# Traneptora/jxlatte

Hardware: AMD Instinct MI355X
Metric: Mpixels/s decoded (VarDCT 4K frame) at 1/2/4/8 MI355X vs host-CPU jxlatte (higher is better)
Workload: dtype f32; 1 GPU; vardct4k: 8 independent 3840x2160 VarDCT frames per GPU (mix=default, Gab + EPF x2 + XYB, f32 out), inputs resident in HBM; frames_per_gpu=8, frames_total=8, frame_seeds=1000 + i, frame i on rank i mod 1, distinct_frames=8, streams=2, kernel_launches_per_frame=2

## Files before the change

jxlatte_amd/csrc/restore_fused_body.h:

```cpp
#pragma once
#include <hip/hip_ext.h>
#include "jxl_internal.h"
#include <algorithm>
#include "restore_sink.h"
#include "epf_quot3.h"
#include <cstdlib>
#include <type_traits>

namespace jxl {

#ifndef JXL_EPF3_PH2_WAVES
#define JXL_EPF3_PH2_WAVES 2
#endif

namespace {

__device__ __forceinline__ int mirror_c(int c, int size) {
    while (c < 0 || c >= size) {
        const int tc = ~c;
        c = tc >= 0 ? tc : (size << 1) + tc;
    }
    return c;
}

template <bool GAB, int ITERS>
struct Geo {
    static constexpr int RG = GAB ? 1 : 0;
    static constexpr int R0 = (ITERS == 3 || ITERS == 4) ? 3 : 0;
    static constexpr int R1 = (ITERS >= 1 && ITERS <= 3) ? 2 : 0;
    static constexpr int R2 = (ITERS == 2 || ITERS == 3) ? 1 : 0;
    static constexpr int SHR = ITERS == 3 ? (R1 + R2) : ITERS == 2 ? R2 : 0;
#ifndef JXL_EPF0_WH
#define JXL_EPF0_WH 64
#endif
    static constexpr int WH = ITERS == 4 ? JXL_EPF0_WH : 32;
    static constexpr int OW = 64 - 2 * SHR, OH = WH - 2 * SHR;
    static constexpr int RE = R0 + R1 + R2;
    static constexpr int RT = RE + RG;
    static constexpr int IW = OW + 2 * RT, IH = OH + 2 * RT;
    static constexpr int SW = IW + 3;
    static constexpr int SH = IH + 1;
    static constexpr int PLANE = SW * SH;
    static constexpr size_t LDS_BYTES = sizeof(float) * (3 * PLANE + 16 * 16);
};

template <int PS>
__device__ __forceinline__ float adiff(const float* p, int u, int v, float s) {
    return u < v ? fabsf(p[u] - p[v]) * s : fabsf(p[v] - p[u]) * s;
}

template <int ITER, int SW, int PLANE, int PH, bool PLAINDIV = false, bool CHAINS = true>
__device__ __forceinline__ void epf_patch(const float* __restrict__ src, int ry, int rx, const float* s_inv ,
                                          const float* bmul , const EpfParams& ep, float res[3][4 * PH]) {
    constexpr int NP = 4 * PH;
    constexpr int R = ITER == 0 ? 3 : ITER == 1 ? 2 : 1;
    constexpr int NW = 4 + 2 * R, NH = PH + 2 * R;
    constexpr int NT = ITER == 0 ? 12 : 4;
    constexpr int TY[12] = {0, 0, -1, 1, -1, 1, 1, -1, 0, 0, 2, -2};
    constexpr int TX[12] = {-1, 1, 0, 0, 1, 1, -1, -1, -2, 2, 0, 0};
    constexpr int QY[5] = {0, 0, 0, -1, 1};
    constexpr int QX[5] = {0, -1, 1, 0, 0};

    float dist[NP][NT];
#pragma unroll
    for (int i = 0; i < NP; i++)
#pragma unroll
        for (int t = 0; t < NT; t++) dist[i][t] = 0.0f;

    if (ITER != 0 && CHAINS) {
        float hc[PH][5], vc[PH + 1][4];
        auto chain_channel = [&](int c, auto first_channel) {
            constexpr bool FIRST = decltype(first_channel)::value;
            float nb[NH * NW];
            const float* pc = src + c * PLANE + (ry - R) * SW + (rx - R);
#pragma unroll
            for (int y = 0; y < NH; y++)
#pragma unroll
                for (int x = 0; x < NW; x++) nb[y * NW + x] = pc[y * SW + x];
            const float sc = ep.channel_scale[c];
#pragma unroll
            for (int py = 0; py < PH; py++)
#pragma unroll
                for (int j = 0; j < 5; j++) {
                    const int cy = py + R, cx = j - 1 + R;
                    if (ITER == 2) {
                        const float t = adiff<NW>(nb, cy * NW + cx, cy * NW + cx + 1, sc);
                        hc[py][j] = FIRST ? t : hc[py][j] + t;
                    } else
#pragma unroll
                        for (int q = 0; q < 5; q++) {
                            const int u = (cy + QY[q]) * NW + cx + QX[q];
                            const float t = adiff<NW>(nb, u, u + 1, sc);
                            hc[py][j] = (FIRST && q == 0) ? t : hc[py][j] + t;
                        }
                }
            constexpr int I0 = 0;
#pragma unroll
            for (int i = I0; i <= PH; i++)
#pragma unroll
                for (int px = 0; px < 4; px++) {
                    const int cy = i - 1 + R, cx = px + R;
                    if (ITER == 2) {
                        const float t = adiff<NW>(nb, cy * NW + cx, (cy + 1) * NW + cx, sc);
                        vc[i][px] = FIRST ? t : vc[i][px] + t;
                    } else
#pragma unroll
                        for (int q = 0; q < 5; q++) {
                            const int u = (cy + QY[q]) * NW + cx + QX[q];
                            const float t = adiff<NW>(nb, u, u + NW, sc);
                            vc[i][px] = (FIRST && q == 0) ? t : vc[i][px] + t;
                        }
                }
        };
        chain_channel(0, std::true_type{});
#pragma unroll 1
        for (int c = 1; c < 3; c++) chain_channel(c, std::false_type{});
#pragma unroll
        for (int py = 0; py < PH; py++)
#pragma unroll
            for (int px = 0; px < 4; px++) {
                dist[py * 4 + px][0] = hc[py][px];
                dist[py * 4 + px][1] = hc[py][px + 1];
                dist[py * 4 + px][2] = vc[py][px];
                dist[py * 4 + px][3] = vc[py + 1][px];
            }
    } else {
    constexpr bool HROW = ITER == 0 && CHAINS && PH == 1;
    float h1[5], h2[6];
#pragma unroll
    for (int j = 0; j < 5; j++) h1[j] = 0.0f;
#pragma unroll
    for (int j = 0; j < 6; j++) h2[j] = 0.0f;
#pragma unroll 1
    for (int c = 0; c < 3; c++) {
        float nb[NH * NW];
        const float* pc = src + c * PLANE + (ry - R) * SW + (rx - R);
#pragma unroll
        for (int y = 0; y < NH; y++)
#pragma unroll
            for (int x = 0; x < NW; x++) nb[y * NW + x] = pc[y * SW + x];
        const float sc = ep.channel_scale[c];
#pragma unroll
        for (int py = 0; py < PH; py++)
#pragma unroll
            for (int px = 0; px < 4; px++) {
                const int cy = py + R, cx = px + R;
#pragma unroll
                for (int t = 0; t < NT; t++) {
                    if (HROW && TY[t] == 0) continue;
                    if (ITER == 2) {
                        dist[py * 4 + px][t] =
                            dist[py * 4 + px][t] + adiff<NW>(nb, cy * NW + cx, (cy + TY[t]) * NW + cx + TX[t], sc);
                    } else {
#pragma unroll
                        for (int q = 0; q < 5; q++) {
                            const int u = (cy + QY[q]) * NW + cx + QX[q];
                            const int v = (cy + TY[t] + QY[q]) * NW + cx + TX[t] + QX[q];
                            dist[py * 4 + px][t] = dist[py * 4 + px][t] + adiff<NW>(nb, u, v, sc);
                        }
                    }
                }
            }
        if (HROW) {
            constexpr int cy = R;
#pragma unroll
            for (int j = 0; j < 5; j++)
#pragma unroll
                for (int q = 0; q < 5; q++) {
                    const int u = (cy + QY[q]) * NW + (j - 1 + R) + QX[q];
                    h1[j] = h1[j] + adiff<NW>(nb, u, u + 1, sc);
                }
#pragma unroll
            for (int j = 0; j < 6; j++)
#pragma unroll
                for (int q = 0; q < 5; q++) {
                    const int u = (cy + QY[q]) * NW + (j - 2 + R) + QX[q];
                    h2[j] = h2[j] + adiff<NW>(nb, u, u + 2, sc);
                }
        }
    }
    if (HROW) {
#pragma unroll
        for (int px = 0; px < 4; px++)
#pragma unroll
            for (int t = 0; t < NT; t++) {
                if (TY[t] != 0) continue;
                dist[px][t] = TX[t] == -1 ? h1[px] : TX[t] == 1 ? h1[px + 1] : TX[t] == -2 ? h2[px] : h2[px + 2];
            }
    }
    }
    float sumW[NP];
    bool skip[NP];
#pragma unroll
    for (int i = 0; i < NP; i++) {
        const float s = s_inv[i];
        skip[i] = (s != s) || (s > (1.0f / 0.3f));
        float sw = 0.0f + 1.0f;
#pragma unroll
        for (int t = 0; t < NT; t++) {
            const float d = dist[i][t] * bmul[i];
            const float v = 1.0f - d * ep.sigma_scale * s;
            const float w = !PLAINDIV ? __builtin_fminf(__builtin_fmaxf(v, 0.0f), 1.0f) : __builtin_fmaxf(v, 0.0f);
            dist[i][t] = w;
            sw = sw + w;
        }
        sumW[i] = sw;
    }
    constexpr int RT2 = ITER == 0 ? 2 : 1;
    constexpr int MW = 4 + 2 * RT2, MH = PH + 2 * RT2;
    if constexpr (!PLAINDIV) {
        float num[3][NP];
#pragma unroll
        for (int c = 0; c < 3; c++) {
            float nb[MH * MW];
            const float* pc = src + c * PLANE + (ry - RT2) * SW + (rx - RT2);
#pragma unroll
            for (int y = 0; y < MH; y++)
#pragma unroll
                for (int x = 0; x < MW; x++) nb[y * MW + x] = pc[y * SW + x];
#pragma unroll
            for (int py = 0; py < PH; py++)
#pragma unroll
                for (int px = 0; px < 4; px++) {
                    const int i = py * 4 + px;
                    const int cy = py + RT2, cx = px + RT2;
                    float sc = 0.0f + nb[cy * MW + cx] * 1.0f;
#pragma unroll
                    for (int t = 0; t < NT; t++) sc = sc + nb[(cy + TY[t]) * MW + cx + TX[t]] * dist[i][t];
                    num[c][i] = sc;
                }
        }
        epf_quot3_patch<NP>(num, sumW, res, [&](int c, int i, float q) {
            const float s = s_inv[i];
            return ((s != s) || (s > (1.0f / 0.3f))) ? src[c * PLANE + (ry + i / 4) * SW + rx + i % 4] : q;
        });
        return;
    }
#pragma unroll
    for (int c = 0; c < 3; c++) {
        float nb[MH * MW];
        const float* pc = src + c * PLANE + (ry - RT2) * SW + (rx - RT2);
#pragma unroll
        for (int y = 0; y < MH; y++)
#pragma unroll
            for (int x = 0; x < MW; x++) nb[y * MW + x] = pc[y * SW + x];
#pragma unroll
        for (int py = 0; py < PH; py++)
#pragma unroll
            for (int px = 0; px < 4; px++) {
                const int i = py * 4 + px;
                const int cy = py + RT2, cx = px + RT2;
                float sc = 0.0f + nb[cy * MW + cx] * 1.0f;
#pragma unroll
                for (int t = 0; t < NT; t++) sc = sc + nb[(cy + TY[t]) * MW + cx + TX[t]] * dist[i][t];
#ifdef JXL_EPF_DIV_BRANCH
                res[c][i] = skip[i] ? nb[cy * MW + cx] : sc / sumW[i];
#else
                float qv = sc / sumW[i];
                asm volatile("" : "+v"(qv));
                res[c][i] = skip[i] ? nb[cy * MW + cx] : qv;
#endif
            }
    }
}

struct TileCtx {
    int ix0, iy0;
    int W, H;
    bool edge;
};

template <int PH, bool EDGE>
__device__ __forceinline__ void patch_sigma(int ry, int rx, const TileCtx& tc, const float* __restrict__ sig, int scy0, int scx0,
                                            const EpfParams& ep, float s_inv[4 * PH], float bmul[4 * PH]) {
    const int gx0 = tc.ix0 + rx;
    int cxa = (gx0 >> 3) - scx0, cxb = ((gx0 + 3) >> 3) - scx0;
    if (EDGE) {
        cxa = (min(max(gx0, 0), tc.W - 1) >> 3) - scx0;
        cxb = (min(max(gx0 + 3, 0), tc.W - 1) >> 3) - scx0;
    }
    const int first_n = 8 - (gx0 & 7);
    const uint32_t colb = 0x8181u >> (gx0 & 7);
#pragma unroll
    for (int py = 0; py < PH; py++) {
        const int gy = tc.iy0 + ry + py;
        const bool rowb = ((gy + 1) & 7) < 2;
        int crow = ((gy >> 3) - scy0) * 16;
        if (EDGE) crow = ((min(max(gy, 0), tc.H - 1) >> 3) - scy0) * 16;
        const float sa = sig[crow + cxa], sb = sig[crow + cxb];
        const uint32_t bm = rowb ? 0xfu : colb;
#pragma unroll
        for (int px = 0; px < 4; px++) {
            bmul[py * 4 + px] = (bm & (1u << px)) ? ep.border_sad_mul : 1.0f;
            s_inv[py * 4 + px] = px < first_n ? sa : sb;
        }
    }
}

template <int ITER, typename G, bool LAST, int PH, bool EDGE, bool PLAINDIV, typename Sink>
__device__ __forceinline__ void epf_stage(float* buf, int m, const TileCtx& tc, const float* __restrict__ sig, int scy0, int scx0,
                                          const EpfParams& ep, Sink sink) {
    constexpr int SW = G::SW, PLANE = G::PLANE;
    const int rw = G::IW - 2 * m, rh = G::IH - 2 * m;
    constexpr int NTHR = 512 / PH;
    const int pcols = (rw + 3) >> 2, prows = (rh + PH - 1) / PH;
    const int cblocks = (pcols + 7) >> 3, n_groups = cblocks * ((prows + 3) >> 2);
    const int q = threadIdx.x & 31;
    auto patch_of = [&](int g, int& prow, int& pcol) {
        pcol = (g % cblocks) * 8 + (q & 7);
        prow = (g / cblocks) * 4 + (q >> 3);
        return prow < prows && pcol < pcols;
    };
    if (LAST) {
        for (int g = threadIdx.x >> 5; g < n_groups; g += NTHR / 32) {
            int prow, pcol;
            if (!patch_of(g, prow, pcol)) continue;
            const int ry = m + prow * PH, rx = m + pcol * 4;
            float s_inv[4 * PH], bmul[4 * PH];
            patch_sigma<PH, EDGE>(ry, rx, tc, sig, scy0, scx0, ep, s_inv, bmul);
            float res[3][4 * PH];
            epf_patch<ITER, SW, PLANE, PH, PLAINDIV>(buf, ry, rx, s_inv, bmul, ep, res);
#pragma unroll
            for (int py = 0; py < PH; py++) {
                const int y = ry + py;
                if (y < G::IH - m) sink.row4(y, rx, &res[0][py * 4], &res[1][py * 4], &res[2][py * 4], min(4, G::IW - m - rx));
            }
        }
    } else {
        static_assert((64 / 4) * ((32 + PH - 1) / PH) <= NTHR, "one patch per thread");
        int prow, pcol;
        const bool act = patch_of(threadIdx.x >> 5, prow, pcol);
        const int ry = m + prow * PH, rx = m + pcol * 4;
        float res[3][4 * PH];
        if (act) {
            float s_inv[4 * PH], bmul[4 * PH];
            patch_sigma<PH, EDGE>(ry, rx, tc, sig, scy0, scx0, ep, s_inv, bmul);
            epf_patch<ITER, SW, PLANE, PH, PLAINDIV>(buf, ry, rx, s_inv, bmul, ep, res);
        }
        __syncthreads();
        if (act) {
#pragma unroll
            for (int py = 0; py < PH; py++) {
                const int y = ry + py;
#pragma unroll
                for (int px = 0; px < 4; px++) {
                    const int x = rx + px;
                    if (y < G::IH - m && x < G::IW - m) {
#pragma unroll
                        for (int c = 0; c < 3; c++) buf[c * PLANE + y * SW + x] = res[c][py * 4 + px];
                    }
                }
            }
        }
    }
}

template <typename G, int NTHR>
__device__ __forceinline__ void mirror_fixup(float* __restrict__ buf, int m, int rem, const TileCtx& tc) {
    const int rw = G::IW - 2 * m, rh = G::IH - 2 * m;
    __syncthreads();
    for (int i = threadIdx.x; i < rw * rh; i += NTHR) {
        const int y = m + i / rw, x = m + i % rw;
        const int gy = tc.iy0 + y, gx = tc.ix0 + x;
        const bool outside = gy < 0 || gy >= tc.H || gx < 0 || gx >= tc.W;
        const bool near = gy >= -rem && gy < tc.H + rem && gx >= -rem && gx < tc.W + rem;
        if (outside && near) {
            const int my = mirror_c(gy, tc.H) - tc.iy0, mx = mirror_c(gx, tc.W) - tc.ix0;
#pragma unroll
            for (int c = 0; c < 3; c++) buf[c * G::PLANE + y * G::SW + x] = buf[c * G::PLANE + my * G::SW + mx];
        }
    }
}


typedef float v2f_t __attribute__((ext_vector_type(2)));
struct __attribute__((packed, aligned(4))) f2a4 {
    float x, y;
};

template <int SK, bool NT = false, bool EDGE = true>
struct OutSink {
    const FusedArgs& a;
    const TileCtx& tc;
    __device__ __forceinline__ void colour(float& v0, float& v1, float& v2) const {
        if (a.p.xyb) invert_xyb_px(a.p.xybp, v0, v1, v2);
    }
    __device__ __forceinline__ void operator()(int y, int x, float v0, float v1, float v2) const {
        const int gy = tc.iy0 + y, gx = tc.ix0 + x;
        if (EDGE && (gy >= tc.H || gx >= tc.W)) return;
        colour(v0, v1, v2);
        sink_store_k<SK>(a, (uint32_t)(gy * tc.W + gx), v0, v1, v2);
    }
    __device__ __forceinline__ void row4(int y, int x, const float* r0, const float* r1, const float* r2, int nvalid) const {
        const int gy = tc.iy0 + y, gx = tc.ix0 + x;
        if (EDGE && gy >= tc.H) return;
        const int n = EDGE ? min(nvalid, tc.W - gx) : nvalid;
        if (n <= 0) return;
        float o[3][4];
#pragma unroll
        for (int i = 0; i < 4; i++) {
            o[0][i] = r0[i];
            o[1][i] = r1[i];
            o[2][i] = r2[i];
            colour(o[0][i], o[1][i], o[2][i]);
        }
        const uint32_t g = (uint32_t)(gy * tc.W + gx);
        if (n == 4 && (g & 1u) == 0 && sink_store4_k<SK, NT>(a, g, o)) return;
#pragma unroll
        for (int i = 0; i < 4; i++)
            if (i < n) sink_store_k<SK>(a, g + i, o[0][i], o[1][i], o[2][i]);
    }
};

template <bool GAB, int ITERS, int SK, int PH, bool EDGE, bool PLAINDIV>
__device__ __forceinline__ void restore_epf_stages(const FusedArgs& a, float* cur, int m, const TileCtx& tc, const float* __restrict__ sig,
                                                   int scy0, int scx0);

template <bool GAB, int ITERS, int SK, int PH, int LAY = 0, bool PLAINDIV = false>
__device__ __forceinline__ void restore_fused_body(const FusedArgs& a) {
    using G = Geo<GAB, ITERS>;
    constexpr int NTHR = 512 / PH;
    extern __shared__ float lds[];
    constexpr int FRONT = LAY == 1 ? 3 : 0;
    float* A = lds + FRONT;
    float* sig = lds + 3 * G::PLANE;
    const int W = a.W, H = a.H;
    TileCtx tc;
    tc.W = W;
    tc.H = H;
    const int tiles_x = (W + G::OW - 1) / G::OW, tiles_y = (H + G::OH - 1) / G::OH;
    int ox, oy;
    {
        const int n_tiles = tiles_x * tiles_y;
        const int per_xcd = (n_tiles + 7) >> 3;
        const int tile = (int)(blockIdx.x & 7u) * per_xcd + (int)(blockIdx.x >> 3);
        if (tile >= n_tiles) return;
        ox = (tile % tiles_x) * G::OW;
        oy = (tile / tiles_x) * G::OH;
    }
    tc.ix0 = ox - G::RT;
    tc.iy0 = oy - G::RT;
    tc.edge = tc.ix0 < 0 || tc.iy0 < 0 || tc.ix0 + G::IW > W || tc.iy0 + G::IH > H;

    const int scy0 = max(tc.iy0, 0) >> 3, scx0 = max(tc.ix0, 0) >> 3;
    if (ITERS > 0 && threadIdx.x < 256) {
        const int cy = scy0 + (threadIdx.x >> 4), cx = scx0 + (threadIdx.x & 15);
        float v = 0.0f;
        if (cy < ((H + 7) >> 3) && cx < a.bw) v = a.inv_sigma[cy * a.bw + cx];
        if (v != v || v > (1.0f / 0.3f)) v = __builtin_inff();
        sig[threadIdx.x] = v;
    }
    if (LAY == 1 && !tc.edge) {
        constexpr int NCX = (G::IW + 6) / 8 + 1, NCY = (G::IH + 6) / 8 + 1, TOTAL = NCX * NCY * 16;
        const int cells_w = W >> 3;
        const int ccy0 = tc.iy0 >> 3, ccx0 = tc.ix0 >> 3;
        static_assert(NTHR % 16 == 0, "a lane keeps its piece index");
        constexpr int CSTEP = NTHR / 16, DY = CSTEP / NCX, DX = CSTEP % NCX;
        const int pc = threadIdx.x & 15;
        const int cyi0 = (int)(threadIdx.x >> 4) / NCX;
        int cxi = (int)(threadIdx.x >> 4) - cyi0 * NCX;
        int y = ((ccy0 + cyi0) << 3) + (pc >> 1) - tc.iy0, x = ((ccx0 + cxi) << 3) + ((pc & 1) << 2) - tc.ix0;
        const size_t tile0 = (size_t)(uint32_t)(ccy0 * cells_w + ccx0) << 6;
        const char* const in0 = reinterpret_cast<const char*>(a.in[0] + tile0);
        const char* const in1 = reinterpret_cast<const char*>(a.in[1] + tile0);
        const char* const in2 = reinterpret_cast<const char*>(a.in[2] + tile0);
        uint32_t g = ((uint32_t)(cyi0 * cells_w + cxi) << 8) + (uint32_t)(pc << 4);
        const uint32_t gstep = (uint32_t)(DY * cells_w + DX) << 8, gwrap = (uint32_t)(cells_w - NCX) << 8;
#pragma unroll
        for (int k = 0; k < (TOTAL + NTHR - 1) / NTHR; k++) {
            if ((unsigned)y < (unsigned)G::IH && (unsigned)(x + 3) < (unsigned)(G::IW + 3)) {
                const float4 v0 = *reinterpret_cast<const float4*>(in0 + g);
                const float4 v1 = *reinterpret_cast<const float4*>(in1 + g);
                const float4 v2 = *reinterpret_cast<const float4*>(in2 + g);
                float* d = A + y * G::SW + x;
                d[0] = v0.x, d[1] = v0.y, d[2] = v0.z, d[3] = v0.w;
                d[G::PLANE] = v1.x, d[G::PLANE + 1] = v1.y, d[G::PLANE + 2] = v1.z, d[G::PLANE + 3] = v1.w;
                d[2 * G::PLANE] = v2.x, d[2 * G::PLANE + 1] = v2.y, d[2 * G::PLANE + 2] = v2.z, d[2 * G::PLANE + 3] = v2.w;
            }
            cxi += DX;
            y += 8 * DY;
            x += 8 * DX;
            g += gstep;
            if (cxi >= NCX) {
                cxi -= NCX;
                y += 8;
                x -= 8 * NCX;
                g += gwrap;
            }
        }
    } else if (!tc.edge) {
        static_assert(G::IW % 2 == 0, "pairs");
        constexpr int PAIRS = G::IW / 2, TOTAL = PAIRS * G::IH;
        const uint32_t base = (uint32_t)(tc.iy0 * W + tc.ix0);
#pragma unroll
        for (int k = 0; k < (TOTAL + NTHR - 1) / NTHR; k++) {
            const int idx = (int)threadIdx.x + k * NTHR;
            if (idx < TOTAL) {
                const int y = idx / PAIRS, x = (idx - y * PAIRS) * 2;
                const uint32_t g = base + (uint32_t)(y * W + x);
                const f2a4 v0 = *reinterpret_cast<const f2a4*>(a.in[0] + g);
                const f2a4 v1 = *reinterpret_cast<const f2a4*>(a.in[1] + g);
                const f2a4 v2 = *reinterpret_cast<const f2a4*>(a.in[2] + g);
                float* d = A + y * G::SW + x;
                d[0] = v0.x;
                d[1] = v0.y;
                d[G::PLANE] = v1.x;
                d[G::PLANE + 1] = v1.y;
                d[2 * G::PLANE] = v2.x;
                d[2 * G::PLANE + 1] = v2.y;
            }
        }
    } else {
        constexpr int STEP_Y = NTHR / G::IW, STEP_X = NTHR % G::IW;
        int y = threadIdx.x / G::IW, x = threadIdx.x % G::IW;
        const float* __restrict__ in0 = a.in[0];
        const float* __restrict__ in1 = a.in[1];
        const float* __restrict__ in2 = a.in[2];
        while (y < G::IH) {
            int gy = tc.iy0 + y, gx = tc.ix0 + x;
            if (GAB) {
                gy = min(max(gy, 0), H - 1);
                gx = min(max(gx, 0), W - 1);
            } else {
                gy = mirror_c(gy, H);
                gx = mirror_c(gx, W);
            }
            const uint32_t g = LAY == 1 ? plane_tiled_off(W >> 3, gy, gx) : (uint32_t)(gy * W + gx);
            const float v0 = in0[g], v1 = in1[g], v2 = in2[g];
            float* d = A + y * G::SW + x;
            d[0] = v0;
            d[G::PLANE] = v1;
            d[2 * G::PLANE] = v2;
            x += STEP_X;
            y += STEP_Y;
            if (x >= G::IW) {
                x -= G::IW;
                y++;
            }
        }
    }
    __syncthreads();
    float* cur = A;
    int m = 0;
    if (GAB) {
        m = 1;
        constexpr int rw = G::IW - 2, rh = G::IH - 2;
        constexpr int NCOLSEG = NTHR / rw;
        constexpr int SEG = (rh + NCOLSEG - 1) / NCOLSEG;
        constexpr int NSEG = (rh + SEG - 1) / SEG;
        static_assert(NSEG * rw <= NTHR, "one pass");
        const int seg = threadIdx.x / rw, x = threadIdx.x - seg * rw;
        const int y0 = seg * SEG;
        float go[3][SEG];
        if (seg < NSEG) {
#pragma unroll
            for (int c = 0; c < 3; c++) {
                const float* p = cur + c * G::PLANE + y0 * G::SW + x;
                float a0 = p[0], a1 = p[1], a2 = p[2];
                float b0 = p[G::SW], b1 = p[G::SW + 1], b2 = p[G::SW + 2];
                float hs_a = a0 + a2;
                const float wb = a.p.gab_base[c], wa = a.p.gab_adj[c], wd = a.p.gab_diag[c];
#pragma unroll
                for (int k = 0; k < SEG; k++) {
                    if (y0 + k < rh) {
                        const float c0 = p[(k + 2) * G::SW], c1 = p[(k + 2) * G::SW + 1], c2 = p[(k + 2) * G::SW + 2];
                        const float hs_b = b0 + b2;
                        const float adj = hs_b + a1 + c1;
                        const float diag = hs_a + c0 + c2;
                        go[c][k] = wb * b1 + wa * adj + wd * diag;
                        a1 = b1;
                        hs_a = hs_b;
                        b0 = c0; b1 = c1; b2 = c2;
                    }
                }
            }
        }
        __syncthreads();
        if (seg < NSEG) {
#pragma unroll
            for (int c = 0; c < 3; c++) {
                float* o = cur + c * G::PLANE + (y0 + 1) * G::SW + x + 1;
#pragma unroll
                for (int k = 0; k < SEG; k++)
                    if (y0 + k < rh) o[k * G::SW] = go[c][k];
            }
        }
        if (tc.edge && ITERS > 0) mirror_fixup<G, NTHR>(cur, m, G::RE, tc);
        __syncthreads();
    }

    if (SK != SK_PLAIN || tc.edge) restore_epf_stages<GAB, ITERS, SK, PH, true, PLAINDIV>(a, cur, m, tc, sig, scy0, scx0);
    else restore_epf_stages<GAB, ITERS, SK, PH, false, PLAINDIV>(a, cur, m, tc, sig, scy0, scx0);
}

template <bool GAB, int ITERS, int SK, int PH, bool EDGE, bool PLAINDIV>
__device__ __forceinline__ void restore_epf_stages(const FusedArgs& a, float* cur, int m, const TileCtx& tc, const float* __restrict__ sig,
                                                   int scy0, int scx0) {
    using G = Geo<GAB, ITERS>;
    constexpr int NTHR = 512 / PH;
    const OutSink<SK, (ITERS != 4), EDGE> sink{a, tc};

    if (ITERS == 0) {
        const int mm = m;
        for (int i = threadIdx.x; i < G::OW * G::OH; i += NTHR) {
            const int y = mm + i / G::OW, x = mm + i % G::OW;
            sink(y, x, cur[y * G::SW + x], cur[G::PLANE + y * G::SW + x], cur[2 * G::PLANE + y * G::SW + x]);
        }
        return;
    }
    if (ITERS == 4) {
        m += 3;
        epf_stage<0, G, true, PH, EDGE, PLAINDIV>(cur, m, tc, sig, scy0, scx0, a.p.epf[0], sink);
        return;
    }
    if (ITERS == 3) {
        m += 3;
        epf_stage<0, G, false, PH, EDGE, PLAINDIV>(cur, m, tc, sig, scy0, scx0, a.p.epf[0], sink);
        if (EDGE) mirror_fixup<G, NTHR>(cur, m, G::R1 + G::R2, tc);
        __syncthreads();
    }
    m += 2;
    if (ITERS >= 2) {
        epf_stage<1, G, false, PH, EDGE, PLAINDIV>(cur, m, tc, sig, scy0, scx0, a.p.epf[1], sink);
        if (EDGE) mirror_fixup<G, NTHR>(cur, m, G::R2, tc);
        __syncthreads();
        m += 1;
        epf_stage<2, G, true, PH, EDGE, PLAINDIV>(cur, m, tc, sig, scy0, scx0, a.p.epf[2], sink);
    } else {
        epf_stage<1, G, true, PH, EDGE, PLAINDIV>(cur, m, tc, sig, scy0, scx0, a.p.epf[1], sink);
    }
}

#define JXL_RESTORE_BOUNDS(ITERS, PH) __launch_bounds__(512 / PH, ITERS >= 3 ? (PH == 1 ? 4 : JXL_EPF3_PH2_WAVES) : PH == 1 ? 8 : 4)
template <bool GAB, int ITERS, int SK, int PH, int LAY = 0, bool PLAINDIV = false>
__global__ JXL_RESTORE_BOUNDS(ITERS, PH) void k_restore_fused(const FusedArgs a) {
    restore_fused_body<GAB, ITERS, SK, PH, LAY, PLAINDIV>(a);
}

template <bool GAB, int ITERS, int SK, bool PLAINDIV = false>
__global__ JXL_RESTORE_BOUNDS(ITERS, 1) void k_restore_fused_batch(const FusedArgs* __restrict__ args) {
    typedef const __attribute__((address_space(4))) FusedArgs* cargs;
    restore_fused_body<GAB, ITERS, SK, 1, 0, PLAINDIV>(*(const FusedArgs*)((cargs)args + blockIdx.y));
}

template <bool GAB, int ITERS, int SK, int PH, int LAY = 0, bool PLAINDIV = false>
void launch_tph(const FusedArgs& a, hipStream_t s) {
    using G = Geo<GAB, ITERS>;
    if constexpr (ITERS > 0 && !PLAINDIV) {
        if (epf_weights_plain(a.p)) return launch_tph<GAB, ITERS, SK, PH, LAY, true>(a, s);
    }
    static const size_t pad = getenv("JXL_RESTORE_LDS_PAD") ? (size_t)atoi(getenv("JXL_RESTORE_LDS_PAD")) : 0;
    static bool attr_set = false;
    if (!attr_set) {
        (void)hipFuncSetAttribute(reinterpret_cast<const void*>(&k_restore_fused<GAB, ITERS, SK, PH, LAY, PLAINDIV>),
                                  hipFuncAttributeMaxDynamicSharedMemorySize, (int)(G::LDS_BYTES + pad));
        attr_set = true;
    }
    const int tiles_x = (a.W + G::OW - 1) / G::OW, tiles_y = (a.H + G::OH - 1) / G::OH;
    const int n_tiles = tiles_x * tiles_y;
    const dim3 grid(((n_tiles + 7) / 8) * 8);
    if (g_restore_kernel_ev[0] && g_restore_kernel_ev[1])
        hipExtLaunchKernelGGL((k_restore_fused<GAB, ITERS, SK, PH, LAY, PLAINDIV>), grid, dim3(512 / PH), (uint32_t)(G::LDS_BYTES + pad), s, g_restore_kernel_ev[0],
                              g_restore_kernel_ev[1], 0u, a);
    else
        hipLaunchKernelGGL((k_restore_fused<GAB, ITERS, SK, PH, LAY, PLAINDIV>), grid, dim3(512 / PH), G::LDS_BYTES + pad, s, a);
}

template <bool GAB, int ITERS, int SK, bool PLAINDIV = false>
void launch_batch_t(const FusedArgs* host_args, const FusedArgs* dev_args, int n, hipStream_t s) {
    using G = Geo<GAB, ITERS>;
    if constexpr (ITERS > 0 && !PLAINDIV) {
        if (epf_weights_plain(host_args[0].p)) return launch_batch_t<GAB, ITERS, SK, true>(host_args, dev_args, n, s);
    }
    static bool attr_set = false;
    if (!attr_set) {
        (void)hipFuncSetAttribute(reinterpret_cast<const void*>(&k_restore_fused_batch<GAB, ITERS, SK, PLAINDIV>),
                                  hipFuncAttributeMaxDynamicSharedMemorySize, (int)G::LDS_BYTES);
        attr_set = true;
    }
    int max_tiles = 0;
    for (int i = 0; i < n; i++)
        max_tiles = std::max(max_tiles, ((host_args[i].W + G::OW - 1) / G::OW) * ((host_args[i].H + G::OH - 1) / G::OH));
    const dim3 grid(((max_tiles + 7) / 8) * 8, n);
    hipLaunchKernelGGL((k_restore_fused_batch<GAB, ITERS, SK, PLAINDIV>), grid, dim3(512), G::LDS_BYTES, s, dev_args);
}

template <int SK>
void launch_fused_sk(const FusedArgs& a, hipStream_t s) {
    const int it = a.p.epf_iters;
    if (a.tiled) {
        if (a.p.gab) {
            if (it == 0) launch_tph<true, 0, SK, 1, 1>(a, s);
            else if (it == 1) launch_tph<true, 1, SK, 1, 1>(a, s);
            else launch_tph<true, 2, SK, 1, 1>(a, s);
        } else {
            if (it == 0) launch_tph<false, 0, SK, 1, 1>(a, s);
            else if (it == 1) launch_tph<false, 1, SK, 1, 1>(a, s);
            else launch_tph<false, 2, SK, 1, 1>(a, s);
        }
        return;
    }
    if (a.p.gab) {
        if (it == 0) launch_tph<true, 0, SK, 1>(a, s);
        else if (it == 1) launch_tph<true, 1, SK, 1>(a, s);
        else if (it == 2) launch_tph<true, 2, SK, 1>(a, s);
        else if (it == 4) {
            if constexpr (SK == SK_PLAIN) launch_tph<true, 4, SK_PLAIN, 1>(a, s);
        } else launch_tph<true, 3, SK, 1>(a, s);
    } else {
        if (it == 0) launch_tph<false, 0, SK, 1>(a, s);
        else if (it == 1) launch_tph<false, 1, SK, 1>(a, s);
        else if (it == 2) launch_tph<false, 2, SK, 1>(a, s);
        else if (it == 4) {
            if constexpr (SK == SK_PLAIN) launch_tph<false, 4, SK_PLAIN, 1>(a, s);
        } else launch_tph<false, 3, SK, 1>(a, s);
    }
}
template <int SK>
void launch_fused_batch_sk(const FusedArgs* h, const FusedArgs* d, int n, hipStream_t s) {
    const int it = h[0].p.epf_iters;
    if (h[0].p.gab) {
        if (it == 0) launch_batch_t<true, 0, SK>(h, d, n, s);
        else if (it == 1) launch_batch_t<true, 1, SK>(h, d, n, s);
        else if (it == 2) launch_batch_t<true, 2, SK>(h, d, n, s);
        else launch_batch_t<true, 3, SK>(h, d, n, s);
    } else {
        if (it == 0) launch_batch_t<false, 0, SK>(h, d, n, s);
        else if (it == 1) launch_batch_t<false, 1, SK>(h, d, n, s);
        else if (it == 2) launch_batch_t<false, 2, SK>(h, d, n, s);
        else launch_batch_t<false, 3, SK>(h, d, n, s);
    }
}

}
}
```

Before: 65130 Mpixels/s.

## Share EPF pair-distance chains between neighbouring patches via LDS and DPP

For the PH==1 EPF iterations 1 and 2, each thread now computes only its own east and south edge-difference chains. It obtains the shared west and north chains from neighbouring lanes through DPP moves, or from a small LDS exchange area at wave and column-group boundaries. The last wave fills the tile-border chains. This removes redundant neighbour-difference arithmetic and register loads per patch, in exchange for extra LDS space, an additional barrier and a fixed thread-to-patch mapping that only holds for this geometry.

```diff
diff --git a/jxlatte_amd/csrc/restore_fused_body.h b/jxlatte_amd/csrc/restore_fused_body.h
--- a/jxlatte_amd/csrc/restore_fused_body.h
+++ b/jxlatte_amd/csrc/restore_fused_body.h
@@ -41,7 +41,10 @@
     static constexpr int SW = IW + 3;
     static constexpr int SH = IH + 1;
     static constexpr int PLANE = SW * SH;
-    static constexpr size_t LDS_BYTES = sizeof(float) * (3 * PLANE + 16 * 16);
+    static constexpr bool HAND = R1 != 0 || R2 != 0;
+    static constexpr int HOFF = (3 * PLANE + 16 * 16 + 3) & ~3;
+    static constexpr int HNORTH = 9 * 64, HWEST = 5 * 32;
+    static constexpr size_t LDS_BYTES = sizeof(float) * (HAND ? HOFF + HNORTH + HWEST : 3 * PLANE + 16 * 16);
 };
 
 template <int PS>
@@ -49,9 +52,83 @@
     return u < v ? fabsf(p[u] - p[v]) * s : fabsf(p[v] - p[u]) * s;
 }
 
-template <int ITER, int SW, int PLANE, int PH, bool PLAINDIV = false, bool CHAINS = true>
+template <int ITER, int SW, int PLANE, int PH, int OWN>
+__device__ __forceinline__ void epf_pair_chains(const float* __restrict__ src, int ry, int rx, const EpfParams& ep, float hc[PH][5],
+                                                float vc[PH + 1][4]) {
+    constexpr int R = ITER == 1 ? 2 : 1;
+    constexpr int NW = 4 + 2 * R, NH = PH + 2 * R;
+    constexpr int QY[5] = {0, 0, 0, -1, 1};
+    constexpr int QX[5] = {0, -1, 1, 0, 0};
+    auto chain_channel = [&](int c, auto first_channel) {
+        constexpr bool FIRST = decltype(first_channel)::value;
+        float nb[NH * NW];
+        const float* pc = src + c * PLANE + (ry - R) * SW + (rx - R);
+#pragma unroll
+        for (int y = 0; y < NH; y++)
+#pragma unroll
+            for (int x = 0; x < NW; x++) nb[y * NW + x] = pc[y * SW + x];
+        const float sc = ep.channel_scale[c];
+#pragma unroll
+        for (int py = 0; py < PH; py++)
+#pragma unroll
+            for (int j = OWN; j < 5; j++) {
+                const int cy = py + R, cx = j - 1 + R;
+                if (ITER == 2) {
+                    const float t = adiff<NW>(nb, cy * NW + cx, cy * NW + cx + 1, sc);
+                    hc[py][j] = FIRST ? t : hc[py][j] + t;
+                } else
+#pragma unroll
+                    for (int q = 0; q < 5; q++) {
+                        const int u = (cy + QY[q]) * NW + cx + QX[q];
+                        const float t = adiff<NW>(nb, u, u + 1, sc);
+                        hc[py][j] = (FIRST && q == 0) ? t : hc[py][j] + t;
+                    }
+            }
+#pragma unroll
+        for (int i = OWN; i <= PH; i++)
+#pragma unroll
+            for (int px = 0; px < 4; px++) {
+                const int cy = i - 1 + R, cx = px + R;
+                if (ITER == 2) {
+                    const float t = adiff<NW>(nb, cy * NW + cx, (cy + 1) * NW + cx, sc);
+                    vc[i][px] = FIRST ? t : vc[i][px] + t;
+                } else
+#pragma unroll
+                    for (int q = 0; q < 5; q++) {
+                        const int u = (cy + QY[q]) * NW + cx + QX[q];
+                        const float t = adiff<NW>(nb, u, u + NW, sc);
+                        vc[i][px] = (FIRST && q == 0) ? t : vc[i][px] + t;
+                    }
+            }
+    };
+    chain_channel(0, std::true_type{});
+#pragma unroll 1
+    for (int c = 1; c < 3; c++) chain_channel(c, std::false_type{});
+}
+
+template <int ITER, int SW, int PLANE, int D>
+__device__ __forceinline__ float epf_pair_chain(const float* __restrict__ src, int y, int x, const EpfParams& ep) {
+    constexpr int QY[5] = {0, 0, 0, -1, 1};
+    constexpr int QX[5] = {0, -1, 1, 0, 0};
+    float d = 0.0f;
+#pragma unroll
+    for (int c = 0; c < 3; c++) {
+        const float* p = src + c * PLANE + y * SW + x;
+        const float sc = ep.channel_scale[c];
+#pragma unroll
+        for (int q = 0; q < (ITER == 2 ? 1 : 5); q++) {
+            const int o = QY[q] * SW + QX[q];
+            const float t = fabsf(p[o] - p[o + D]) * sc;
+            d = (c == 0 && q == 0) ? t : d + t;
+        }
+    }
+    return d;
+}
+
+template <int ITER, int SW, int PLANE, int PH, bool PLAINDIV = false, bool CHAINS = true, bool GIVEN = false>
 __device__ __forceinline__ void epf_patch(const float* __restrict__ src, int ry, int rx, const float* s_inv ,
-                                          const float* bmul , const EpfParams& ep, float res[3][4 * PH]) {
+                                          const float* bmul , const EpfParams& ep, float res[3][4 * PH],
+                                          const float* given_h = nullptr , const float* given_v = nullptr ) {
     constexpr int NP = 4 * PH;
     constexpr int R = ITER == 0 ? 3 : ITER == 1 ? 2 : 1;
     constexpr int NW = 4 + 2 * R, NH = PH + 2 * R;
@@ -69,52 +146,15 @@
 
     if (ITER != 0 && CHAINS) {
         float hc[PH][5], vc[PH + 1][4];
-        auto chain_channel = [&](int c, auto first_channel) {
-            constexpr bool FIRST = decltype(first_channel)::value;
-            float nb[NH * NW];
-            const float* pc = src + c * PLANE + (ry - R) * SW + (rx - R);
-#pragma unroll
-            for (int y = 0; y < NH; y++)
-#pragma unroll
-                for (int x = 0; x < NW; x++) nb[y * NW + x] = pc[y * SW + x];
-            const float sc = ep.channel_scale[c];
-#pragma unroll
-            for (int py = 0; py < PH; py++)
-#pragma unroll
-                for (int j = 0; j < 5; j++) {
-                    const int cy = py + R, cx = j - 1 + R;
-                    if (ITER == 2) {
-                        const float t = adiff<NW>(nb, cy * NW + cx, cy * NW + cx + 1, sc);
-                        hc[py][j] = FIRST ? t : hc[py][j] + t;
-                    } else
-#pragma unroll
-                        for (int q = 0; q < 5; q++) {
-                            const int u = (cy + QY[q]) * NW + cx + QX[q];
-                            const float t = adiff<NW>(nb, u, u + 1, sc);
-                            hc[py][j] = (FIRST && q == 0) ? t : hc[py][j] + t;
-                        }
-                }
-            constexpr int I0 = 0;
-#pragma unroll
-            for (int i = I0; i <= PH; i++)
-#pragma unroll
-                for (int px = 0; px < 4; px++) {
-                    const int cy = i - 1 + R, cx = px + R;
-                    if (ITER == 2) {
-                        const float t = adiff<NW>(nb, cy * NW + cx, (cy + 1) * NW + cx, sc);
-                        vc[i][px] = FIRST ? t : vc[i][px] + t;
-                    } else
-#pragma unroll
-                        for (int q = 0; q < 5; q++) {
-                            const int u = (cy + QY[q]) * NW + cx + QX[q];
-                            const float t = adiff<NW>(nb, u, u + NW, sc);
-                            vc[i][px] = (FIRST && q == 0) ? t : vc[i][px] + t;
-                        }
-                }
-        };
-        chain_channel(0, std::true_type{});
-#pragma unroll 1
-        for (int c = 1; c < 3; c++) chain_channel(c, std::false_type{});
+        if constexpr (GIVEN) {
+            static_assert(PH == 1, "exchanged chains: 4x1 patches");
+#pragma unroll
+            for (int j = 0; j < 5; j++) hc[0][j] = given_h[j];
+#pragma unroll
+            for (int px = 0; px < 4; px++) vc[0][px] = given_v[px], vc[1][px] = given_v[4 + px];
+        } else {
+            epf_pair_chains<ITER, SW, PLANE, PH, 0>(src, ry, rx, ep, hc, vc);
+        }
 #pragma unroll
         for (int py = 0; py < PH; py++)
 #pragma unroll
@@ -304,6 +344,64 @@
     const int rw = G::IW - 2 * m, rh = G::IH - 2 * m;
     constexpr int NTHR = 512 / PH;
     const int pcols = (rw + 3) >> 2, prows = (rh + PH - 1) / PH;
+    if constexpr (PH == 1 && ITER != 0) {
+        static_assert(!G::HAND || (G::OW > 48 && G::WH == 32 && NTHR == 512), "13..16 patch columns, 32 window rows on 8 waves");
+        extern __shared__ __attribute__((aligned(16))) float lds[];
+        float* const hnorth = lds + G::HOFF;
+        float* const hwest = hnorth + G::HNORTH;
+        const int lane = threadIdx.x & 63, wave = threadIdx.x >> 6;
+        const int pcol = ((lane >> 4) << 2) + (lane & 3), prow = (wave << 2) + ((lane >> 2) & 3);
+        const bool act = prow < prows && pcol < pcols;
+        const int ry = m + prow, rx = m + pcol * 4;
+        constexpr int R = ITER == 1 ? 2 : 1;
+        const bool whole = !PLAINDIV && m + 31 + R <= G::IH && m + 63 + R <= G::IW + 2;
+        float s_inv[4], bmul[4];
+        float hc[5], vc[2][4];
+        if (whole || act) {
+            patch_sigma<1, EDGE>(ry, rx, tc, sig, scy0, scx0, ep, s_inv, bmul);
+            float (*h1)[5] = reinterpret_cast<float (*)[5]>(hc);
+            epf_pair_chains<ITER, SW, PLANE, 1, 1>(buf, ry, rx, ep, h1, vc);
+            if ((lane & 12) == 12) {
+                float* d = hnorth + (wave + 1) * 64 + pcol * 4;
+                *reinterpret_cast<float4*>(d) = make_float4(vc[1][0], vc[1][1], vc[1][2], vc[1][3]);
+            }
+            if ((lane & 3) == 3) hwest[((pcol >> 2) + 1) * 32 + prow] = hc[4];
+        }
+        if (__builtin_amdgcn_readfirstlane(wave) == NTHR / 64 - 1) {
+            if (lane < rw) hnorth[lane] = epf_pair_chain<ITER, SW, PLANE, SW>(buf, m - 1, m + lane, ep);
+            if (lane < rh) hwest[lane] = epf_pair_chain<ITER, SW, PLANE, 1>(buf, m + lane, m - 1, ep);
+        }
+        __syncthreads();
+        float res[3][4];
+        if (whole || act) {
+            const float4 n4 = *reinterpret_cast<const float4*>(hnorth + wave * 64 + pcol * 4);
+            const float w1 = hwest[(pcol >> 2) * 32 + prow];
+            const float nn[4] = {n4.x, n4.y, n4.z, n4.w};
+#pragma unroll
+            for (int px = 0; px < 4; px++)
+                vc[0][px] = __int_as_float(
+                    __builtin_amdgcn_update_dpp(__float_as_int(nn[px]), __float_as_int(vc[1][px]), 0x114, 0xf, 0xf, false));
+            const float wl = __int_as_float(__builtin_amdgcn_mov_dpp(__float_as_int(hc[4]), 0x90, 0xf, 0xf, true));
+            hc[0] = (lane & 3) == 0 ? w1 : wl;
+            epf_patch<ITER, SW, PLANE, 1, PLAINDIV, true, true>(buf, ry, rx, s_inv, bmul, ep, res, hc, &vc[0][0]);
+        }
+        if constexpr (LAST) {
+            if (act) sink.row4(ry, rx, &res[0][0], &res[1][0], &res[2][0], min(4, G::IW - m - rx));
+        } else {
+            __syncthreads();
+            if (act) {
+#pragma unroll
+                for (int px = 0; px < 4; px++) {
+                    const int x = rx + px;
+                    if (x < G::IW - m) {
+#pragma unroll
+                        for (int c = 0; c < 3; c++) buf[c * PLANE + ry * SW + x] = res[c][px];
+                    }
+                }
+            }
+        }
+        return;
+    }
     const int cblocks = (pcols + 7) >> 3, n_groups = cblocks * ((prows + 3) >> 2);
     const int q = threadIdx.x & 31;
     auto patch_of = [&](int g, int& prow, int& pcol) {
@@ -420,7 +518,7 @@
 __device__ __forceinline__ void restore_fused_body(const FusedArgs& a) {
     using G = Geo<GAB, ITERS>;
     constexpr int NTHR = 512 / PH;
-    extern __shared__ float lds[];
+    extern __shared__ __attribute__((aligned(16))) float lds[];
     constexpr int FRONT = LAY == 1 ? 3 : 0;
     float* A = lds + FRONT;
     float* sig = lds + 3 * G::PLANE;
```

Result: faster. 66860 Mpixels/s (median of 6 runs) (+2.7%).
